# SHI-Labs/Self-Similarity-Grouping

Measured on AMD Instinct MI355X. Metric: images/s embed + s/iter for NxN rerank+DBSCAN, N=16k, 1/2/4/8 GPU, higher is better.
Workload: dtype f32 (embed: split-half operands hi+lo on fp16 MFMA, fp32 accumulate, 6e-8 max error vs the fp32 reference features) / exact int64 via int8 MFMA digits + f64 + f16 (distance, re-rank: half semantics, bit-exact)

## Files before the change

include/ssg_hip.h:

```cpp
#ifndef SSG_HIP_H
#define SSG_HIP_H

#include <stddef.h>
#include <stdint.h>

#ifdef __cplusplus
extern "C" {
#endif

typedef struct ihipStream_t* ssg_stream_t;

#define SSG_OK 0
#define SSG_ERR_INVALID (-1)
#define SSG_ERR_HIP (-2)
#define SSG_ERR_OVERFLOW (-3)
#define SSG_ERR_NAN (-4)

const char* ssg_last_error(void);
int ssg_version(void);
uint16_t ssg_double_to_half_bits(double d);

int ssg_range_stats_f32(const float* a, int rows_a, const float* b, int rows_b, int d, float* out4, ssg_stream_t stream);
int ssg_row_norms_f64(const float* x, int n, int d, int round_to_half, double* norms, ssg_stream_t stream);
int ssg_sqdist_self_f16(const float* x, const double* norms, int N, int d, int row0, int nrows, int memory_save, uint16_t* D, uint32_t* rowmax,
// ... 87 lines not shown
                           const int64_t* seg_off, const int32_t* seg_len, int nseg, const uint64_t* s_cursor, const uint32_t* vmin,
                           uint16_t jp0_half, uint8_t* rowmask, int32_t* cnt, int32_t* edges, uint64_t cap_edges, uint64_t* cursor2,
                           ssg_stream_t stream);
int ssg_concat_segments_u64(const uint64_t* in, int nseg, uint64_t seg_cap, uint64_t seg_stride, const uint64_t* counts, int count_stride,
                            uint64_t* out, uint64_t* total2, ssg_stream_t stream);
size_t ssg_dbscan_cc_workspace_bytes(int N);
int ssg_dbscan_cc(const int32_t* cnt, const int32_t* edges, uint64_t nedges, int N, int min_samples, void* ws, size_t ws_bytes,
                  int64_t* labels, ssg_stream_t stream);
int ssg_dbscan_cc_dev(const int32_t* cnt, const int32_t* edges, const uint64_t* nedges_dev, uint64_t cap_edges, int N, int min_samples,
                      void* ws, size_t ws_bytes, int64_t* labels, ssg_stream_t stream);

int ssg_conv2d_nhwc_f32(const float* in, const float* w, const float* bias, const float* res, float* out, int B, int H, int W, int Cin,
                        int Cout, int KH, int KW, int stride, int pad, int relu, ssg_stream_t stream);
int ssg_conv1x1_dual_nhwc_f32(const float* in, const float* in2, const float* w, const float* bias, float* out, int B, int H, int W, int Cin,
                              int H2, int W2, int Cin2, int stride2, int Cout, int relu, ssg_stream_t stream);
#define SSG_CONV_IN_SPLIT 1
#define SSG_CONV_OUT_SPLIT 2
int ssg_conv2d_nhwc_x(const void* in, const void* w, const float* bias, const void* res, void* out, int B, int H, int W, int Cin,
                      int Cout, int KH, int KW, int stride, int pad, int relu, int flags, float acc_scale, const float* ch_scale,
                      int32_t* overflow, ssg_stream_t stream);
int ssg_conv1x1_dual_nhwc_x(const void* in, const void* in2, const void* w, const float* bias, void* out, int B, int H, int W, int Cin,
                            int H2, int W2, int Cin2, int stride2, int Cout, int relu, int flags, float acc_scale, const float* ch_scale,
                            int32_t* overflow, ssg_stream_t stream);
int ssg_conv_pair_supported(int K1, int C, int N2);
int ssg_conv_pair_nhwc_x(const void* y2, const void* w3, const float* b3, const float* cs3, const void* res, void* out,
                         const void* w1n, const float* b1n, const float* cs1n, void* y1n, int M, int K1, int C, int N2,
                         int32_t* overflow, ssg_stream_t stream);
int ssg_bottleneck_supported(int H, int W, int CIN, int C, int MID);
int ssg_bottleneck_nhwc_x(const void* x, const void* w1, const float* b1, const float* cs1, const void* w2, const float* b2, const float* cs2,
                          const void* w3, const float* b3, const float* cs3, void* out, int B, int H, int W, int C, int MID,
                          int32_t* overflow, ssg_stream_t stream);
int ssg_bottleneck_ds_nhwc_x(const void* x, const void* w1, const float* b1, const float* cs1, const void* w2, const float* b2, const float* cs2,
                             const void* w3cat, const float* b3, const float* cs3, void* out, int B, int H, int W, int CIN, int C, int MID,
                             int32_t* overflow, ssg_stream_t stream);
int ssg_basicblock_supported(int H, int W, int C);
int ssg_basicblock_nhwc_x(const void* x, const void* w1, const float* b1, const float* cs1, const void* w2, const float* b2, const float* cs2,
                          void* out, int B, int H, int W, int C, int32_t* overflow, ssg_stream_t stream);
int ssg_stem_pool_supported(int H, int W);
int ssg_stem_pool_nchw_x(const float* images, int flip, const void* w, const float* bias, const float* ch_scale, void* out, int B, int H, int W,
                         int32_t* overflow, ssg_stream_t stream);
int ssg_nchw_to_nhwc4_h4l4(const float* in, void* out, int B, int H, int W, int flip, ssg_stream_t stream);
int ssg_maxpool3x3s2_h8l8(const void* in, void* out, int B, int H, int W, int C, ssg_stream_t stream);
int ssg_gap_stripes_h8l8(const void* in, float* out, int B, int H, int W, int C, int num_split, ssg_stream_t stream);
int ssg_h8l8_encode(const float* in, void* out, int64_t n, float scale, ssg_stream_t stream);
int ssg_h8l8_decode(const void* in, float* out, int64_t n, float scale, ssg_stream_t stream);
int ssg_pairwise_sqdist_f32(const float* x, const float* y, int m, int n, int d, int self_form, float* ws, float* out, ssg_stream_t stream);
// ... 179 lines not shown
```

self-similarity-grouping_amd/csrc/conv.hip:

```cpp
#include "ssg_common.h"
#include <cstdlib>
#include <type_traits>

namespace ssg {

typedef float v16f __attribute__((ext_vector_type(16)));
typedef unsigned int v4u __attribute__((ext_vector_type(4)));
typedef _Float16 v8h __attribute__((ext_vector_type(8)));

__device__ __forceinline__ unsigned pack_h2(_Float16 a, _Float16 b) {
  return (unsigned)__builtin_bit_cast(unsigned short, a) | ((unsigned)__builtin_bit_cast(unsigned short, b) << 16);
}
__device__ __forceinline__ float unpack_lo(unsigned u) { return (float)__builtin_bit_cast(_Float16, (unsigned short)(u & 0xffffu)); }
__device__ __forceinline__ float unpack_hi(unsigned u) { return (float)__builtin_bit_cast(_Float16, (unsigned short)(u >> 16)); }
__device__ __forceinline__ void split_encode4(const float4 v, uint2& hi, uint2& lo) {
  const _Float16 h0 = (_Float16)v.x, h1 = (_Float16)v.y, h2 = (_Float16)v.z, h3 = (_Float16)v.w;
  hi = make_uint2(pack_h2(h0, h1), pack_h2(h2, h3));
  lo = make_uint2(pack_h2((_Float16)(v.x - (float)h0), (_Float16)(v.y - (float)h1)), pack_h2((_Float16)(v.z - (float)h2), (_Float16)(v.w - (float)h3)));
}
__device__ __forceinline__ bool split_hi_nonfinite(const uint2 hi) {
  const unsigned a = hi.x & 0x7fff7fffu, b = hi.y & 0x7fff7fffu;
  return (a & 0xffffu) >= 0x7c00u || (a >> 16) >= 0x7c00u || (b & 0xffffu) >= 0x7c00u || (b >> 16) >= 0x7c00u;
}
__device__ __forceinline__ float4 split_decode4(const uint2 hi, const uint2 lo) {
  return make_float4(unpack_lo(hi.x) + unpack_lo(lo.x), unpack_hi(hi.x) + unpack_hi(lo.x), unpack_lo(hi.y) + unpack_lo(lo.y), unpack_hi(hi.y) + unpack_hi(lo.y));
}

struct ConvParams {
  const float* in; const float* w; const float* bias; const float* res; float* out;
  int B, H, W, Cin, OH, OW, Cout, KH, KW, stride, pad, relu;
  int M, Kpad;
  int variant;
  unsigned in_bytes;
  const float* in2; int H2, W2, Cin2, stride2, nk1; unsigned in2_bytes;
  const float* rowterm; int epi;
  float* tilemin; int tmin_ld;
  int out_split, res_split; float acc_scale;
  const float* cscale = nullptr;
  int* overflow = nullptr;
  int products = 3;
  unsigned long long* prof = nullptr;
};
#ifdef SSG_DMA_PROF
#define SSG_DMA_STAMP(I_) { if (p.prof && threadIdx.x == 0) p.prof[(size_t)blockIdx.x * 8 + (I_)] = __builtin_readcyclecounter(); }
#else
#define SSG_DMA_STAMP(I_)
#endif

constexpr int CLD32 = 36;

__device__ __forceinline__ int conv_xcd_remap(int b, int nwg) {
  const int nx = 8, q = nwg / nx, r = nwg % nx, x = b % nx, s = b / nx;
  return (x < r ? x * (q + 1) : r * (q + 1) + (x - r) * q) + s;
}

template <int MT, int NT> struct SplitFrags { v8h ah[MT], al[MT], bh[NT], bl[NT]; };

typedef float v4f __attribute__((ext_vector_type(4)));
template <int MT, int NT, int CLD, bool TAP4>
__device__ __forceinline__ void split_load_frags(const float* Arow, const float* Brow, const int kofs, SplitFrags<MT, NT>& f) {
#pragma unroll
  for (int i = 0; i < MT; i++) {
    const float* q = Arow + i * 32 * CLD + kofs;
// ... 406 lines not shown
  const int wm = wave / WCOLS, wn = wave % WCOLS, l32 = lane & 31, h = lane >> 5;

  const int drow = lane >> 2, pc = lane & 3;
  const int lc4 = (pc ^ ((drow >> 2) & 3)) * 4;
  const int nkA = DUAL ? p.nk1 * 2 : 0x7fffffff;
  int ab0, ah0, aw0, ab1 = -1, ah1 = 0, aw1 = 0, abase0 = 0, abase1 = 0;
  unsigned a2b0 = 0x80000000u, a2b1 = 0x80000000u;
#define SSG_ROW(J)                                                                                                   \
  {                                                                                                                  \
    const int m = tm * BM + (wave * ABLK + J) * 16 + drow;                                                            \
    if (m < p.M) {                                                                                                   \
      const int b = m / (p.OH * p.OW), rem = m - b * (p.OH * p.OW);                                                  \
      const int oh = rem / p.OW, ow = rem - oh * p.OW;                                                               \
      ab##J = b; ah##J = oh * p.stride - p.pad; aw##J = ow * p.stride - p.pad;                                       \
      abase##J = (((b * p.H + ah##J) * p.W + aw##J) * p.Cin + lc4) * 4;                                               \
      if (DUAL) a2b##J = (unsigned)((((b * p.H2 + oh * p.stride2) * p.W2 + ow * p.stride2) * p.Cin2 + lc4) * 4);       \
    } else { ab##J = -1; ah##J = 0; aw##J = 0; }                                                                     \
  }
  SSG_ROW(0)
  if (ABLK == 2) SSG_ROW(1)
#undef SSG_ROW
  const __amdgpu_buffer_rsrc_t in_rsrc = __builtin_amdgcn_make_buffer_rsrc(const_cast<float*>(p.in), 0, p.in_bytes, 0x00020000);
  const __amdgpu_buffer_rsrc_t in2_rsrc = __builtin_amdgcn_make_buffer_rsrc(const_cast<float*>(p.in2 ? p.in2 : p.in), 0, p.in2 ? p.in2_bytes : 0u, 0x00020000);
  const __amdgpu_buffer_rsrc_t w_rsrc = __builtin_amdgcn_make_buffer_rsrc(const_cast<float*>(p.w), 0, (unsigned)((int64_t)p.Cout * p.Kpad * 4), 0x00020000);
  const unsigned wo0 = (unsigned)(((tn * BN + wave * (16 * WBLK) + drow) * p.Kpad + lc4) * 4), wo1 = wo0 + (unsigned)(16 * p.Kpad * 4);
  const int nk = p.Kpad / CBK;
  int dn = 0, dr = 0, ds = 0, dch = 0;
#ifndef SSG_DMA_AUX_A
#define SSG_DMA_AUX_A 0
#endif
#ifndef SSG_DMA_AUX_W
#define SSG_DMA_AUX_W 0
#endif
#define SSG_DMA_A(J, ST)                                                                                             \
  {                                                                                                                  \
    if (!DUAL || dn < nkA) {                                                                                          \
      const bool ok = ab##J >= 0 && (unsigned)(ah##J + dr) < (unsigned)p.H && (unsigned)(aw##J + ds) < (unsigned)p.W;  \
      const unsigned aoff = ok ? (unsigned)(abase##J + ddelta_) : 0x80000000u;                                        \
      __builtin_amdgcn_raw_ptr_buffer_load_lds(in_rsrc, SSG_LDSP(ST + (wave * ABLK + J) * 1024), 16, aoff, 0, 0, SSG_DMA_AUX_A);   \
    } else {                                                                                                          \
      const unsigned aoff = a2b##J + (unsigned)((dn - nkA) * CBK * 4);                                                 \
      __builtin_amdgcn_raw_ptr_buffer_load_lds(in2_rsrc, SSG_LDSP(ST + (wave * ABLK + J) * 1024), 16, aoff, 0, 0, SSG_DMA_AUX_A);  \
    }                                                                                                                 \
  }
#define SSG_DMA_NEXT(ST)                                                                                             \
  {                                                                                                                  \
    const int ddelta_ = ((dr * p.W + ds) * p.Cin + dch * 32 + (dn & 1) * 16) * 4;                                     \
    SSG_DMA_A(0, ST) if (ABLK == 2) SSG_DMA_A(1, ST)                                                                  \
    const unsigned kb_ = (unsigned)(dn * CBK * 4);                                                                    \
    __builtin_amdgcn_raw_ptr_buffer_load_lds(w_rsrc, SSG_LDSP(ST + BM * 64 + wave * (1024 * WBLK)), 16, wo0 + kb_, 0, 0, SSG_DMA_AUX_W);   \
    if (WBLK == 2) __builtin_amdgcn_raw_ptr_buffer_load_lds(w_rsrc, SSG_LDSP(ST + BM * 64 + wave * 2048 + 1024), 16, wo1 + kb_, 0, 0, SSG_DMA_AUX_W); \
    {                                         \
      const int adv_ = dn < nk - 1 ? 1 : 0;                                                                          \
      dn += adv_;                                                                                                    \
      ds += adv_ & ~dn & 1;                                                                                          \
      const int w1_ = ds == p.KW ? 1 : 0; ds = w1_ ? 0 : ds; dr += w1_;                                               \
      const int w2_ = dr == p.KH ? 1 : 0; dr = w2_ ? 0 : dr; dch += w2_;                                              \
    }                                                                                                                \
  }

  const int g = (l32 >> 2) & 3;
  const int offh = ((2 * h) ^ g) * 16, offl = ((2 * h + 1) ^ g) * 16;
  const int arow = (wm * WM + l32) * 64, brow = BM * 64 + (wn * WN + l32) * 64;
#define SSG_MMA(ST)                                                                                                  \
  {                                                                                                                  \
    v8h ah_[MT], al_[MT], bh_[NT], bl_[NT];                                                                          \
    _Pragma("unroll") for (int i = 0; i < MT; i++) {                                                                 \
      ah_[i] = *reinterpret_cast<const v8h*>(ST + arow + i * 2048 + offh); al_[i] = *reinterpret_cast<const v8h*>(ST + arow + i * 2048 + offl); } \
    _Pragma("unroll") for (int j = 0; j < NT; j++) {                                                                 \
      bh_[j] = *reinterpret_cast<const v8h*>(ST + brow + j * 2048 + offh); bl_[j] = *reinterpret_cast<const v8h*>(ST + brow + j * 2048 + offl); } \
    if constexpr (!ONEPROD) {                                                                                        \
      _Pragma("unroll") for (int i = 0; i < MT; i++) _Pragma("unroll") for (int j = 0; j < NT; j++)                  \
// ... 310 lines not shown
            const unsigned s0 = odd ? __float_as_uint(r4.x) : __float_as_uint(r4.z), s1 = odd ? __float_as_uint(r4.y) : __float_as_uint(r4.w);
            const unsigned g0 = lane_xor1(s0), g1 = lane_xor1(s1);
            r4 = odd ? split_decode4(make_uint2(g0, g1), make_uint2(__float_as_uint(r4.z), __float_as_uint(r4.w)))
                     : split_decode4(make_uint2(__float_as_uint(r4.x), __float_as_uint(r4.y)), make_uint2(g0, g1));
          }
          v.x += r4.x; v.y += r4.y; v.z += r4.z; v.w += r4.w;
        }
        if (p.relu) { v.x = v.x > 0.f ? v.x : 0.f; v.y = v.y > 0.f ? v.y : 0.f; v.z = v.z > 0.f ? v.z : 0.f; v.w = v.w > 0.f ? v.w : 0.f; }
        if (p.out_split) {
          uint2 hp, lp;
          split_encode4(v, hp, lp);
          if (p.overflow && split_hi_nonfinite(hp)) *p.overflow = 1;
          const uint2 send = odd ? hp : lp;
          const uint2 recv = make_uint2(lane_xor1(send.x), lane_xor1(send.y));
          const uint4 stv = odd ? make_uint4(recv.x, recv.y, lp.x, lp.y) : make_uint4(hp.x, hp.y, recv.x, recv.y);
          if (m < p.M) *reinterpret_cast<uint4*>(outp + (int64_t)m * p.Cout + col) = stv;
        } else if (m < p.M) *reinterpret_cast<float4*>(outp + (int64_t)m * p.Cout + col) = v;
      }
      __builtin_amdgcn_fence(__ATOMIC_ACQ_REL, "wavefront");
    }
  }
}

__global__ void nchw_to_nhwc4_kernel(const float* __restrict__ in, float* __restrict__ out, int B, int H, int W, int flip) {
  const int64_t total = (int64_t)B * H * W;
  for (int64_t x = (int64_t)blockIdx.x * blockDim.x + threadIdx.x; x < total; x += (int64_t)gridDim.x * blockDim.x) {
    const int w = (int)(x % W); const int64_t t = x / W; const int hh = (int)(t % H); const int b = (int)(t / H);
    const int ws = flip ? (W - 1 - w) : w;
    const int64_t plane = (int64_t)H * W, base = (int64_t)b * 3 * plane + (int64_t)hh * W + ws;
    reinterpret_cast<float4*>(out)[x] = make_float4(in[base], in[base + plane], in[base + 2 * plane], 0.f);
  }
}

__global__ void nchw_to_nhwc4_h4l4_kernel(const float* __restrict__ in, float* __restrict__ out, int B, int H, int W, int flip) {
  const int64_t total = (int64_t)B * H * W;
  for (int64_t x = (int64_t)blockIdx.x * blockDim.x + threadIdx.x; x < total; x += (int64_t)gridDim.x * blockDim.x) {
    const int w = (int)(x % W); const int64_t t = x / W; const int hh = (int)(t % H); const int b = (int)(t / H);
    const int ws = flip ? (W - 1 - w) : w;
    const int64_t plane = (int64_t)H * W, base = (int64_t)b * 3 * plane + (int64_t)hh * W + ws;
    uint2 hi, lo;
    split_encode4(make_float4(in[base], in[base + plane], in[base + 2 * plane], 0.f), hi, lo);
    reinterpret_cast<uint4*>(out)[x] = make_uint4(hi.x, hi.y, lo.x, lo.y);
  }
}

__global__ void maxpool3x3s2_kernel(const float* __restrict__ in, float* __restrict__ out, int B, int H, int W, int C, int OH, int OW) {
// ... 183 lines not shown
      if (tall_wm == 128) hipLaunchKernelGGL((conv_dma_kernel<256, false, 256, false, 4, 128, false>), dim3(tiles_tall), dim3(512), 0, stream, p);
      else if (tall_wm == 129) hipLaunchKernelGGL((conv_dma_kernel<256, false, 256, false, 4, 128, true>), dim3(tiles_tall), dim3(512), 0, stream, p);
      else if (tall_ns == 4) hipLaunchKernelGGL((conv_dma_kernel<256, false, 256, false, 4>), dim3(tiles_tall), dim3(1024), 0, stream, p);
      else hipLaunchKernelGGL((conv_dma_kernel<256, false, 256, false>), dim3(tiles_tall), dim3(1024), 0, stream, p);
      return ssg_check_hip(hipGetLastError(), "conv_dma_kernel<256x256>");
    }
    const int tiles = ((p.M + 127) / 128) * (p.Cout / 256);
    if (p.products == 1) hipLaunchKernelGGL((conv_dma_kernel<256, true>), dim3(tiles), dim3(512), 0, stream, p);
    else if (p.in2) hipLaunchKernelGGL((conv_dma_kernel<256, false, 128, true>), dim3(tiles), dim3(512), 0, stream, p);
    else hipLaunchKernelGGL(conv_dma_kernel<256>, dim3(tiles), dim3(512), 0, stream, p);
    return ssg_check_hip(hipGetLastError(), "conv_dma_kernel");
  }
  return launch_conv_bk<128, 256, 64, 64, false, 32, true>(p, stream);
}

static bool conv_prefers_bn64(const ConvParams& p, bool split) {
  static int maxtiles = -1;
  if (maxtiles < 0) { const char* e = getenv("SSG_SPLIT_BN64_MAXTILES"); maxtiles = e ? atoi(e) : 300; }
  if (!split) return false;
  const int tiles = ((p.M + 127) / 128) * (p.Cout / 128);
  return tiles < maxtiles;
}

extern "C" int ssg_conv2d_nhwc_x(const void* in, const void* w, const float* bias, const void* res, void* out, int B, int H, int W,
                                 int Cin, int Cout, int KH, int KW, int stride, int pad, int relu, int flags, float acc_scale, const float* ch_scale,
                                 int32_t* overflow, hipStream_t stream) {
  ConvParams p;
  p.cscale = ch_scale; p.overflow = overflow;
  p.in = (const float*)in; p.w = (const float*)w; p.bias = bias; p.res = (const float*)res; p.out = (float*)out;
  p.B = B; p.H = H; p.W = W; p.Cin = Cin; p.Cout = Cout; p.KH = KH; p.KW = KW; p.stride = stride; p.pad = pad; p.relu = relu;
  p.OH = (H + 2 * pad - KH) / stride + 1; p.OW = (W + 2 * pad - KW) / stride + 1;
  const int64_t M = (int64_t)B * p.OH * p.OW;
  const bool split = (flags & 1) != 0;
  if (B <= 0 || M <= 0 || M > 0x7fffffff || (Cout % 64) || !((Cin % 32) == 0 || Cin == 4) || stride < 1) {
    ssg_set_error("ssg_conv2d_nhwc: unsupported shape B=%d H=%d W=%d Cin=%d Cout=%d k=%dx%d s=%d p=%d flags=%d", B, H, W, Cin, Cout, KH, KW, stride, pad, flags);
    return SSG_ERR_INVALID;
  }
  p.M = (int)M;
  const int64_t in_bytes = (int64_t)B * H * W * Cin * 4;
  if (in_bytes > 0x7fffffffLL) { ssg_set_error("ssg_conv2d_nhwc: input tensor of %lld bytes exceeds the 2 GiB buffer-resource range of this kernel; use a smaller batch", (long long)in_bytes); return SSG_ERR_INVALID; }
  p.in_bytes = (unsigned)in_bytes;
  p.in2 = nullptr; p.H2 = p.W2 = p.Cin2 = 0; p.stride2 = 1; p.in2_bytes = 0; p.rowterm = nullptr; p.epi = 0; p.tilemin = nullptr; p.tmin_ld = 0;
  p.out_split = (flags & 2) ? 1 : 0; p.res_split = p.out_split; p.acc_scale = acc_scale;
  static int variant = -1;
  if (variant < 0) { const char* e = getenv("SSG_CONV_VARIANT"); variant = e ? atoi(e) : 0; }
  p.variant = variant;
  const bool cin4 = (Cin == 4);
  p.Kpad = cin4 ? 32 * ((KH * KW + 7) / 8) : KH * KW * Cin;
  p.nk1 = p.Kpad / 16;
  if (cin4) return (Cout % 128 == 0) ? launch_conv<128, 128, 64, 64, true>(p, stream, split) : launch_conv<128, 64, 64, 32, true>(p, stream, split);
  if (conv_prefers_wide(p, split)) return launch_conv_wide(p, stream);
  return (Cout % 128 == 0 && !conv_prefers_bn64(p, split)) ? launch_conv<128, 128, 64, 64, false>(p, stream, split) : launch_conv<128, 64, 64, 32, false>(p, stream, split);
}

extern "C" int ssg_conv2d_nhwc_f32(const float* in, const float* w, const float* bias, const float* res, float* out, int B, int H, int W,
                                   int Cin, int Cout, int KH, int KW, int stride, int pad, int relu, hipStream_t stream) {
  return ssg_conv2d_nhwc_x(in, w, bias, res, out, B, H, W, Cin, Cout, KH, KW, stride, pad, relu, 0, 1.f, nullptr, nullptr, stream);
}

extern "C" int ssg_conv1x1_dual_nhwc_x(const void* in, const void* in2, const void* w, const float* bias, void* out, int B, int H, int W,
                                       int Cin, int H2, int W2, int Cin2, int stride2, int Cout, int relu, int flags, float acc_scale, const float* ch_scale,
                                       int32_t* overflow, hipStream_t stream) {
  ConvParams p;
  p.cscale = ch_scale; p.overflow = overflow;
  p.in = (const float*)in; p.w = (const float*)w; p.bias = bias; p.res = nullptr; p.out = (float*)out;
  p.B = B; p.H = H; p.W = W; p.Cin = Cin; p.Cout = Cout; p.KH = 1; p.KW = 1; p.stride = 1; p.pad = 0; p.relu = relu;
  p.OH = H; p.OW = W;
  const int64_t M = (int64_t)B * H * W;
  const int64_t in_bytes = M * Cin * 4, in2_bytes = (int64_t)B * H2 * W2 * Cin2 * 4;
  if (B <= 0 || M > 0x7fffffff || (Cout % 64) || (Cin % 32) || (Cin2 % 32) || stride2 < 1 || (H - 1) * stride2 >= H2 || (W - 1) * stride2 >= W2 ||
      in_bytes > 0x7fffffffLL || in2_bytes > 0x7fffffffLL) {
    ssg_set_error("ssg_conv1x1_dual_nhwc: unsupported shape B=%d H=%d W=%d Cin=%d H2=%d W2=%d Cin2=%d s2=%d Cout=%d", B, H, W, Cin, H2, W2, Cin2, stride2, Cout);
    return SSG_ERR_INVALID;
  }
  p.M = (int)M; p.in_bytes = (unsigned)in_bytes;
  p.in2 = (const float*)in2; p.H2 = H2; p.W2 = W2; p.Cin2 = Cin2; p.stride2 = stride2; p.in2_bytes = (unsigned)in2_bytes;
  p.Kpad = Cin + Cin2; p.nk1 = Cin / 32; p.variant = 0; p.rowterm = nullptr; p.epi = 0; p.tilemin = nullptr; p.tmin_ld = 0;
  p.out_split = (flags & 2) ? 1 : 0; p.res_split = p.out_split; p.acc_scale = acc_scale;
  const bool split = (flags & 1) != 0;
  if (conv_prefers_wide(p, split)) return launch_conv_wide(p, stream);
  return (Cout % 128 == 0 && !conv_prefers_bn64(p, split)) ? launch_conv<128, 128, 64, 64, false>(p, stream, split) : launch_conv<128, 64, 64, 32, false>(p, stream, split);
}

extern "C" int ssg_conv1x1_dual_nhwc_f32(const float* in, const float* in2, const float* w, const float* bias, float* out, int B, int H, int W,
                                         int Cin, int H2, int W2, int Cin2, int stride2, int Cout, int relu, hipStream_t stream) {
  return ssg_conv1x1_dual_nhwc_x(in, in2, w, bias, out, B, H, W, Cin, H2, W2, Cin2, stride2, Cout, relu, 0, 1.f, nullptr, nullptr, stream);
}

namespace ssg {
__global__ __launch_bounds__(256) void row_sqnorm_kernel(const float* __restrict__ x, int rows, int d, float scale, float* __restrict__ out) {
  const int row = (int)((blockIdx.x * blockDim.x + threadIdx.x) >> 6);
  if (row >= rows) return;
  const int lane = lane_id();
  float s = 0.f;
  const float* xr = x + (int64_t)row * d;
  for (int c0 = lane; c0 < d; c0 += 512) {
    float v[8];
#pragma unroll
    for (int u = 0; u < 8; u++) v[u] = xr[min(c0 + 64 * u, d - 1)];
#pragma unroll
    for (int u = 0; u < 8; u++) if (c0 + 64 * u < d) s += v[u] * v[u];
  }
  for (int sh = 1; sh < 64; sh <<= 1) s += __shfl_xor(s, sh, 64);
  if (lane == 0) out[row] = s * scale;
// ... 98 lines not shown
```

self-similarity-grouping_amd/resnet.py:

```python
from collections import OrderedDict

import math
import os

import torch

from . import _lib
from ._lib import check, ptr, stream

_LAYERS = {18: (2, 2, 2, 2), 34: (3, 4, 6, 3), 50: (3, 4, 6, 3), 101: (3, 4, 23, 3), 152: (3, 8, 36, 3)}
_BASIC = (18, 34)
_BN_EPS = 1e-5
_DEC_CLUSTERS, _DEC_DIM, _DEC_KEY = 32, 2048, "assignment.cluster_centers"
_FUSED_BASICBLOCK_DEFAULT = "1"


def _expansion(depth):
    return 1 if depth in _BASIC else 4


def _arch(depth):
    blocks = []
    inplanes = 64
    exp = _expansion(depth)
# ... 35 lines not shown
            conv(p + ".conv2", pl, pl, 3); bn(p + ".bn2", pl)
            if blk["down"]:
                conv(p + ".downsample.0", pl, ip, 1); bn(p + ".downsample.1", pl)
            continue
        conv(p + ".conv1", pl, ip, 1); bn(p + ".bn1", pl)
        conv(p + ".conv2", pl, pl, 3); bn(p + ".bn2", pl)
        conv(p + ".conv3", pl * 4, pl, 1); bn(p + ".bn3", pl * 4)
        if blk["down"]:
            conv(p + ".downsample.0", pl * 4, ip, 1); bn(p + ".downsample.1", pl * 4)
    sd["base.fc.weight"] = torch.randn(1000, width, generator=g) * 0.01
    sd["base.fc.bias"] = torch.zeros(1000)
    if num_features > 0:
        sd["feat.weight"] = torch.randn(num_features, width, generator=g) * 0.001
        sd["feat_bn.weight"] = torch.ones(num_features); sd["feat_bn.bias"] = torch.zeros(num_features)
        sd["feat_bn.running_mean"] = torch.zeros(num_features); sd["feat_bn.running_var"] = torch.ones(num_features)
        sd["feat_bn.num_batches_tracked"] = torch.zeros((), dtype=torch.long)
    if cluster:
        bound = math.sqrt(6.0 / (_DEC_CLUSTERS + _DEC_DIM))
        sd[_DEC_KEY] = (torch.rand(_DEC_CLUSTERS, _DEC_DIM, generator=g) * 2.0 - 1.0) * bound
    return sd


class _FoldedConv:
    __slots__ = ("w", "bias", "cin", "cout", "k", "stride", "pad", "split", "acc_scale", "cscale")


_IN_SPLIT, _OUT_SPLIT = 1, 2


def _h8l8(v):
    rows, K = v.shape
    hi = v.half()
    lo = (v - hi.float()).half()
    g = torch.stack([hi.view(rows, K // 8, 8), lo.view(rows, K // 8, 8)], dim=2)
    return g.reshape(rows, 2 * K).contiguous().view(torch.float32)


def _h4l4(v):
    rows, K = v.shape
    hi = v.half()
    lo = (v - hi.float()).half()
    g = torch.stack([hi.view(rows, K // 4, 4), lo.view(rows, K // 4, 4)], dim=2)
    return g.reshape(rows, 2 * K).contiguous().view(torch.float32)


def _weight_scale(w):
    mx = float(w.abs().max())
    return 256.0 if mx == 0 else float(min(256.0, 2.0 ** math.floor(math.log2(16384.0 / mx))))


# ... 15 lines not shown
    mean, var = sd[bn_name + ".running_mean"].double(), sd[bn_name + ".running_var"].double()
    scale = gamma / torch.sqrt(var + _BN_EPS)
    w = w * scale.view(-1, 1, 1, 1)
    bias = beta - mean * scale
    cout, cin, k, _ = w.shape
    w = w.permute(0, 2, 3, 1).contiguous()
    if cin == 3:
        w = torch.nn.functional.pad(w, (0, 1))
        cin = 4
        kpad = 32 * ((k * k + 7) // 8)
        w = torch.nn.functional.pad(w.reshape(cout, k * k * 4), (0, kpad - k * k * 4))
    else:
        w = pack_weight_khwc(w)
    f = _FoldedConv()
    w = w.float().contiguous()
    f.split, f.acc_scale, f.cscale = bool(split), 1.0, None
    if split:
        sc = _row_scales(w)
        w = w * sc.view(-1, 1)
        w = _h4l4(w) if cin == 4 else _h8l8(w)
        f.cscale = (1.0 / sc).contiguous().to(device)
    f.w = w.to(device); f.bias = bias.float().contiguous().to(device)
    f.cin, f.cout, f.k, f.stride, f.pad = cin, cout, k, stride, pad
    return f


def _fold_mode():
    return os.environ.get("SSG_DEVICE_FOLD", "")


def _bn_keys(conv_name, bn_name):
    return (conv_name + ".weight", bn_name + ".weight", bn_name + ".bias", bn_name + ".running_mean", bn_name + ".running_var")


def _use_device_fold(sd, keys):
    mode = _fold_mode()
    return mode == "1" or (mode != "0" and any(sd[k].device.type != "cpu" for k in keys))


def _fold_device(sources, stride, pad, device, split=False):
    L = _lib.lib()
    srcs = [[t.detach().to(device, torch.float32) for t in s] for s in sources]
    w = srcs[0][0]
    cout, cin, k, kw = w.shape
    f = _FoldedConv()
    f.split, f.acc_scale, f.cscale = bool(split), 1.0, None
    kp = 32 * ((k * kw + 7) // 8) if cin == 3 else sum(s[0].shape[1] * s[0].shape[2] * s[0].shape[3] for s in srcs)
    f.w = torch.empty((cout, kp), dtype=torch.float32, device=device)
    f.bias = torch.empty(cout, dtype=torch.float32, device=device)
    if split:
        f.cscale = torch.empty(cout, dtype=torch.float32, device=device)
    if len(srcs) == 1:
        g, b, m, v = srcs[0][1:]
        st = w.stride()
        check(L.ssg_fold_conv_bn_f32(ptr(w), st[0], st[1], st[2], st[3], cout, cin, k, kw, ptr(g), ptr(b), ptr(m), ptr(v), _BN_EPS, 1 if split else 0,
                                     ptr(f.w), ptr(f.bias), ptr(f.cscale), stream()), "ssg_fold_conv_bn_f32")
    else:
        args = []
        for wt, g, b, m, v in srcs:
            st = wt.stride()
            args += [ptr(wt), st[0], st[1], st[2], st[3], wt.shape[1], wt.shape[2], wt.shape[3], ptr(g), ptr(b), ptr(m), ptr(v)]
        check(L.ssg_fold_conv_bn_dual_f32(*args, _BN_EPS, cout, 1 if split else 0, ptr(f.w), ptr(f.bias), ptr(f.cscale), stream()),
              "ssg_fold_conv_bn_dual_f32")
    last = srcs[-1][0]
    f.cin, f.cout, f.k, f.stride, f.pad = (4 if cin == 3 else last.shape[1]), cout, last.shape[2], stride, pad
    return f


class ResNet:

    def __init__(self, depth=50, checkpoint=None, pretrained=True, num_features=2048, dropout=0.1, num_classes=0, num_split=1,
                 mode='Dissimilarity', cluster=False, seed=1, precision=None):
        if depth not in _LAYERS:
            raise KeyError("Unsupported depth:", depth)
        if num_classes > 0:
            raise NotImplementedError("num_classes > 0 (dropout + classifier head, resnet.py:118-120) is a training-only path; "
                                      "the grouping path uses num_classes=0 (selftraining.py:121-123)")
        if num_features > 0 and num_features % 64:
            raise ValueError("num_features must be a multiple of 64")
        self.depth, self.num_features, self.dropout, self.num_classes = depth, num_features, dropout, num_classes
        self.out_planes = 512 * _expansion(depth)
        self.num_split, self.cluster, self.pretrained, self.training = num_split, cluster, pretrained, False
        self.precision = precision or os.environ.get("SSG_EMBED_PRECISION", "split")
        if self.precision not in ("split", "f32"):
            raise ValueError("precision must be 'split' or 'f32'")
        self.device = torch.device("cpu")
        self._sd = synthetic_state_dict(seed, depth, num_features, cluster=bool(cluster))
        self._folded = None
        self._twin = None
        self.flip_streams = True
        self._weights = "synthetic"
        if checkpoint:
            self.load_state_dict(torch.load(checkpoint, map_location="cpu"), strict=False)
        elif pretrained:
            import warnings
            warnings.warn("ssg_amd ResNet(pretrained=True): no ImageNet weights are available offline; the backbone holds seeded "
                          "synthetic weights until load_state_dict()/checkpoint= supplies real ones", stacklevel=2)

    def state_dict(self):
        return OrderedDict((k, v.clone() if v.device.type == "cpu" else v.cpu()) for k, v in self._sd.items())

    def load_state_dict(self, state_dict, strict=True):
        state_dict, missing, unexpected = self._match_keys(state_dict, strict)
        for k, v in state_dict.items():
            if k in self._sd:
                if tuple(v.shape) != tuple(self._sd[k].shape):
                    raise RuntimeError("size mismatch for %s: %r vs %r" % (k, tuple(v.shape), tuple(self._sd[k].shape)))
                self._sd[k] = v.detach().to("cpu").clone()
        self._invalidate()
        self._report_missing("load_state_dict", missing)
        return missing, unexpected

# ... 68 lines not shown
    def _host_sd(self, keys):
        return {k: self._sd[k].cpu() for k in keys}

    def _fold_one(self, conv_name, bn_name, stride, pad, split=False):
        keys = _bn_keys(conv_name, bn_name)
        if _use_device_fold(self._sd, keys):
            return _fold_device([[self._sd[k] for k in keys]], stride, pad, self.device, split=split)
        return _fold(self._host_sd(keys), conv_name, bn_name, stride, pad, self.device, split=split)

    def _fold_dual(self, p, stride, sp):
        dev = self.device
        k3, kd = _bn_keys(p + ".conv3", p + ".bn3"), _bn_keys(p + ".downsample.0", p + ".downsample.1")
        if _use_device_fold(self._sd, k3 + kd):
            c3 = _fold_device([[self._sd[k] for k in k3]], 1, 0, dev)
            ds = _fold_device([[self._sd[k] for k in k3], [self._sd[k] for k in kd]], stride, 0, dev, split=sp)
            return c3, ds
        sd = self._host_sd(k3 + kd)
        c3 = _fold(sd, p + ".conv3", p + ".bn3", 1, 0, dev)
        ds = _fold(sd, p + ".downsample.0", p + ".downsample.1", stride, 0, dev)
        wcat = torch.cat([c3.w, ds.w], dim=1)
        if sp:
            sc = _row_scales(wcat.cpu())
            ds.w = _h8l8((wcat.cpu() * sc.view(-1, 1))).to(dev); ds.acc_scale = 1.0; ds.cscale = (1.0 / sc).contiguous().to(dev); ds.split = True
        else:
            ds.w = wcat.contiguous()
        ds.bias = (c3.bias + ds.bias).contiguous()
        return c3, ds

    def _prepare(self):
        if self._folded is not None:
            return self._folded
        if self.device.type != "cuda":
            raise _lib.SSGError("the embedder runs on the GPU only: call model.cuda() first (no CPU fallback)")
        sp = self.precision == "split"
        fold = self._fold_one
        net = dict(stem=fold("base.conv1", "base.bn1", 2, 3, sp), blocks=[], split=sp)
        for blk in _arch(self.depth):
            p = blk["prefix"]
            if blk["kind"] == "basic":
                net["blocks"].append(dict(
                    kind="basic",
                    c1=fold(p + ".conv1", p + ".bn1", blk["stride"], 1, sp),
                    c2=fold(p + ".conv2", p + ".bn2", 1, 1, sp),
                    ds=fold(p + ".downsample.0", p + ".downsample.1", blk["stride"], 0, sp) if blk["down"] else None))
                continue
            if blk["down"]:
                c3, ds = self._fold_dual(p, blk["stride"], sp)
            else:
                c3, ds = fold(p + ".conv3", p + ".bn3", 1, 0, sp), None
            net["blocks"].append(dict(
                c1=fold(p + ".conv1", p + ".bn1", 1, 0, sp),
                c2=fold(p + ".conv2", p + ".bn2", blk["stride"], 1, sp),
                c3=c3, ds=ds))
        self._folded = net
        return net

    @staticmethod
    def _conv(L, x, f, res=None, relu=True, out_split=False, ovf=None):
        B, H, W, _ = x.shape
        OH = (H + 2 * f.pad - f.k) // f.stride + 1; OW = (W + 2 * f.pad - f.k) // f.stride + 1
        out = torch.empty((B, OH, OW, f.cout), dtype=torch.float32, device=x.device)
        flags = (_IN_SPLIT if f.split else 0) | (_OUT_SPLIT if out_split else 0)
        check(L.ssg_conv2d_nhwc_x(ptr(x), ptr(f.w), ptr(f.bias), ptr(res), ptr(out), B, H, W, f.cin, f.cout, f.k, f.k, f.stride, f.pad,
                                  1 if relu else 0, flags, f.acc_scale, ptr(getattr(f, "cscale", None)), ptr(ovf), stream()), "ssg_conv2d_nhwc_x")
        return out

    @staticmethod
    def _conv_dual(L, o, x, c3, ds, out_split=False, ovf=None):
        B, H, W, _ = o.shape
        _, H2, W2, _ = x.shape
        out = torch.empty((B, H, W, c3.cout), dtype=torch.float32, device=o.device)
        flags = (_IN_SPLIT if ds.split else 0) | (_OUT_SPLIT if out_split else 0)
        check(L.ssg_conv1x1_dual_nhwc_x(ptr(o), ptr(x), ptr(ds.w), ptr(ds.bias), ptr(out), B, H, W, c3.cin, H2, W2, ds.cin, ds.stride, c3.cout, 1,
                                        flags, ds.acc_scale, ptr(getattr(ds, "cscale", None)), ptr(ovf), stream()), "ssg_conv1x1_dual_nhwc_x")
        return out

    @staticmethod
    def _bottleneck(L, y, blk, ovf=None):
        B, H, W, CIN = y.shape
        c1, c2, c3, ds = blk["c1"], blk["c2"], blk["c3"], blk["ds"]
        if os.environ.get("SSG_FUSED_BOTTLENECK", "1") == "0" or c2.stride != 1 or (ds is not None and ds.stride != 1):
            return None
        if not L.ssg_bottleneck_supported(H, W, CIN, c3.cout, c1.cout):
            return None
        out = torch.empty((B, H, W, c3.cout), dtype=torch.float32, device=y.device)
        if ds is None:
            check(L.ssg_bottleneck_nhwc_x(ptr(y), ptr(c1.w), ptr(c1.bias), ptr(c1.cscale), ptr(c2.w), ptr(c2.bias), ptr(c2.cscale),
                                          ptr(c3.w), ptr(c3.bias), ptr(c3.cscale), ptr(out), B, H, W, CIN, c1.cout, ptr(ovf), stream()),
                  "ssg_bottleneck_nhwc_x")
        else:
            check(L.ssg_bottleneck_ds_nhwc_x(ptr(y), ptr(c1.w), ptr(c1.bias), ptr(c1.cscale), ptr(c2.w), ptr(c2.bias), ptr(c2.cscale),
                                             ptr(ds.w), ptr(ds.bias), ptr(ds.cscale), ptr(out), B, H, W, CIN, c3.cout, c1.cout, ptr(ovf), stream()),
                  "ssg_bottleneck_ds_nhwc_x")
        return out

    @staticmethod
    def _basicblock(L, y, blk, ovf=None):
        B, H, W, C = y.shape
        c1, c2 = blk["c1"], blk["c2"]
        if os.environ.get("SSG_FUSED_BASICBLOCK", _FUSED_BASICBLOCK_DEFAULT) == "0" or c1.stride != 1 or blk["ds"] is not None or c1.cout != C:
            return None
        if not L.ssg_basicblock_supported(H, W, C):
            return None
        out = torch.empty((B, H, W, C), dtype=torch.float32, device=y.device)
        check(L.ssg_basicblock_nhwc_x(ptr(y), ptr(c1.w), ptr(c1.bias), ptr(c1.cscale), ptr(c2.w), ptr(c2.bias), ptr(c2.cscale), ptr(out),
                                      B, H, W, C, ptr(ovf), stream()), "ssg_basicblock_nhwc_x")
        return out

    def _fmap(self, x, flip=False, hooks=None):
        L = _lib.lib()
        net = self._prepare()
        sp = net["split"]
        x = x.to(self.device, torch.float32).contiguous()
        B, C, H, W = x.shape
        if C != 3:
            raise ValueError("expected RGB images [B,3,H,W]")
        ovf = self._overflow_flag() if sp else None
        if sp and os.environ.get("SSG_FUSED_STEM", "1") != "0" and L.ssg_stem_pool_supported(H, W):
            st = net["stem"]
            y = torch.empty((B, H // 4, W // 4, 64), dtype=torch.float32, device=self.device)
            check(L.ssg_stem_pool_nchw_x(ptr(x), 1 if flip else 0, ptr(st.w), ptr(st.bias), ptr(st.cscale), ptr(y), B, H, W, ptr(ovf), stream()),
                  "ssg_stem_pool_nchw_x")
        else:
            x4 = torch.empty((B, H, W, 4), dtype=torch.float32, device=self.device)
            if sp:
                check(L.ssg_nchw_to_nhwc4_h4l4(ptr(x), ptr(x4), B, H, W, 1 if flip else 0, stream()), "ssg_nchw_to_nhwc4_h4l4")
            else:
                check(L.ssg_nchw_to_nhwc4(ptr(x), ptr(x4), B, H, W, 1 if flip else 0, stream()), "ssg_nchw_to_nhwc4")
            y = self._conv(L, x4, net["stem"], out_split=sp, ovf=ovf)
            _, H2, W2, _ = y.shape
            p = torch.empty((B, (H2 + 1) // 2, (W2 + 1) // 2, 64), dtype=torch.float32, device=self.device)
            if sp:
                check(L.ssg_maxpool3x3s2_h8l8(ptr(y), ptr(p), B, H2, W2, 64, stream()), "ssg_maxpool3x3s2_h8l8")
            else:
                check(L.ssg_maxpool3x3s2_nhwc(ptr(y), ptr(p), B, H2, W2, 64, stream()), "ssg_maxpool3x3s2_nhwc")
            y = p
        pair = sp and os.environ.get("SSG_CONV_PAIR", "0") == "1"
        blocks, o1_next = net["blocks"], None
        for bi, blk in enumerate(blocks):
            if hooks and bi in hooks:
                hooks[bi]()
            if blk.get("kind") == "basic":
                fused = self._basicblock(L, y, blk, ovf) if sp else None
                if fused is not None:
                    y = fused
                    continue
                o = self._conv(L, y, blk["c1"], out_split=sp, ovf=ovf)
                r = y if blk["ds"] is None else self._conv(L, y, blk["ds"], relu=False, out_split=sp, ovf=ovf)
                y = self._conv(L, o, blk["c2"], res=r, relu=True, out_split=sp, ovf=ovf)
                continue
            if sp:
                fused = self._bottleneck(L, y, blk, ovf)
                if fused is not None:
                    y = fused
                    continue
            o = o1_next if o1_next is not None else self._conv(L, y, blk["c1"], out_split=sp, ovf=ovf)
            o1_next = None
            o = self._conv(L, o, blk["c2"], out_split=sp, ovf=ovf)
            if blk["ds"] is not None:
                y = self._conv_dual(L, o, y, blk["c3"], blk["ds"], out_split=sp, ovf=ovf)
                continue
            nxt = blocks[bi + 1]["c1"] if bi + 1 < len(blocks) else None
            Bo, Ho, Wo, _ = o.shape
            if (pair and nxt is not None and nxt.k == 1 and nxt.stride == 1 and nxt.cin == blk["c3"].cout and Bo * Ho * Wo >= 128 * 256
                    and L.ssg_conv_pair_supported(blk["c3"].cin, blk["c3"].cout, nxt.cout)):
                y, o1_next = self._conv_pair(L, o, blk["c3"], y, nxt, ovf)
            else:
                y = self._conv(L, o, blk["c3"], res=y, relu=True, out_split=sp, ovf=ovf)
        return y, sp

    @staticmethod
    def _conv_pair(L, o, c3, res, c1n, ovf=None):
        B, H, W, _ = o.shape
        out = torch.empty((B, H, W, c3.cout), dtype=torch.float32, device=o.device)
        y1n = torch.empty((B, H, W, c1n.cout), dtype=torch.float32, device=o.device)
        check(L.ssg_conv_pair_nhwc_x(ptr(o), ptr(c3.w), ptr(c3.bias), ptr(c3.cscale), ptr(res), ptr(out), ptr(c1n.w), ptr(c1n.bias), ptr(c1n.cscale),
                                     ptr(y1n), B * H * W, c3.cin, c3.cout, c1n.cout, ptr(ovf), stream()), "ssg_conv_pair_nhwc_x")
        return out, y1n

    def _side_streams(self):
        st = getattr(self, "_streams", None)
        if st is None or st[0].device != self.device:
            prio = -1 if os.environ.get("SSG_FLIP_PRIO", "0") == "1" else 0
            st = self._streams = (torch.cuda.Stream(self.device, priority=prio), torch.cuda.Stream(self.device))
        return st

    def _overflow_flag(self):
        if getattr(self, "_ovf", None) is None or self._ovf.device != self.device:
            self._ovf = torch.zeros(1, dtype=torch.int32, device=self.device)
        return self._ovf

# ... 157 lines not shown
```

Before: 27860.

## Pre-tile conv weights into swizzled 128-row K-tile blocks for contiguous DMA loads

Adds a one-time kernel that rearranges split-half conv weights into 128-output-channel by K-tile blocks, with an XOR swizzle on the 16-byte columns. The conv kernel reads this copy through the buffer-to-LDS loads, so each wave fetches one contiguous 1 KiB chunk per K step instead of strided rows. The tiled copy sits right after the original weights in one allocation, and the python path sets a flag so the kernel finds it at w + Cout*Kpad. This costs double the weight memory and a tiling pass at fold time, and only applies to split-half weights with Cout divisible by 128.

```diff
diff --git a/include/ssg_hip.h b/include/ssg_hip.h
--- a/include/ssg_hip.h
+++ b/include/ssg_hip.h
@@ -133,6 +133,15 @@
 int ssg_conv1x1_dual_nhwc_x(const void* in, const void* in2, const void* w, const float* bias, void* out, int B, int H, int W, int Cin,
                             int H2, int W2, int Cin2, int stride2, int Cout, int relu, int flags, float acc_scale, const float* ch_scale,
                             int32_t* overflow, ssg_stream_t stream);
+#define SSG_CONV_W_TILED 4
+int ssg_conv_weights_tile_supported(int Cout, int Kpad);
+int ssg_conv_weights_tile(const void* w, int Cout, int Kpad, void* wt, ssg_stream_t stream);
+int ssg_conv2d_nhwc_xt(const void* in, const void* w, const void* wt, const float* bias, const void* res, void* out, int B, int H, int W, int Cin,
+                       int Cout, int KH, int KW, int stride, int pad, int relu, int flags, float acc_scale, const float* ch_scale,
+                       int32_t* overflow, ssg_stream_t stream);
+int ssg_conv1x1_dual_nhwc_xt(const void* in, const void* in2, const void* w, const void* wt, const float* bias, void* out, int B, int H, int W, int Cin,
+                             int H2, int W2, int Cin2, int stride2, int Cout, int relu, int flags, float acc_scale, const float* ch_scale,
+                             int32_t* overflow, ssg_stream_t stream);
 int ssg_conv_pair_supported(int K1, int C, int N2);
 int ssg_conv_pair_nhwc_x(const void* y2, const void* w3, const float* b3, const float* cs3, const void* res, void* out,
                          const void* w1n, const float* b1n, const float* cs1n, void* y1n, int M, int K1, int C, int N2,
diff --git a/self-similarity-grouping_amd/csrc/conv.hip b/self-similarity-grouping_amd/csrc/conv.hip
--- a/self-similarity-grouping_amd/csrc/conv.hip
+++ b/self-similarity-grouping_amd/csrc/conv.hip
@@ -39,6 +39,7 @@
   const float* cscale = nullptr;
   int* overflow = nullptr;
   int products = 3;
+  const float* wt = nullptr;
   unsigned long long* prof = nullptr;
 };
 #ifdef SSG_DMA_PROF
@@ -491,9 +492,16 @@
 #undef SSG_ROW
   const __amdgpu_buffer_rsrc_t in_rsrc = __builtin_amdgcn_make_buffer_rsrc(const_cast<float*>(p.in), 0, p.in_bytes, 0x00020000);
   const __amdgpu_buffer_rsrc_t in2_rsrc = __builtin_amdgcn_make_buffer_rsrc(const_cast<float*>(p.in2 ? p.in2 : p.in), 0, p.in2 ? p.in2_bytes : 0u, 0x00020000);
-  const __amdgpu_buffer_rsrc_t w_rsrc = __builtin_amdgcn_make_buffer_rsrc(const_cast<float*>(p.w), 0, (unsigned)((int64_t)p.Cout * p.Kpad * 4), 0x00020000);
-  const unsigned wo0 = (unsigned)(((tn * BN + wave * (16 * WBLK) + drow) * p.Kpad + lc4) * 4), wo1 = wo0 + (unsigned)(16 * p.Kpad * 4);
+#ifndef SSG_CONV_WT
+#define SSG_CONV_WT 1
+#endif
   const int nk = p.Kpad / CBK;
+  const bool tiled = SSG_CONV_WT && !ONEPROD && p.wt != nullptr;
+  const __amdgpu_buffer_rsrc_t w_rsrc = __builtin_amdgcn_make_buffer_rsrc(const_cast<float*>(tiled ? p.wt : p.w), 0, (unsigned)((int64_t)p.Cout * p.Kpad * 4), 0x00020000);
+  const int wrow0 = tn * BN + wave * (16 * WBLK);
+  const unsigned wo0 = tiled ? (unsigned)((((wrow0 >> 7) * nk) * 128 + (wrow0 & 127)) * 64 + lane * 16) : (unsigned)(((wrow0 + drow) * p.Kpad + lc4) * 4);
+  const unsigned wo1 = wo0 + (tiled ? 1024u : (unsigned)(16 * p.Kpad * 4));
+  const int wkshift = tiled ? 13 : 6;
   int dn = 0, dr = 0, ds = 0, dch = 0;
 #ifndef SSG_DMA_AUX_A
 #define SSG_DMA_AUX_A 0
@@ -516,7 +524,7 @@
   {                                                                                                                  \
     const int ddelta_ = ((dr * p.W + ds) * p.Cin + dch * 32 + (dn & 1) * 16) * 4;                                     \
     SSG_DMA_A(0, ST) if (ABLK == 2) SSG_DMA_A(1, ST)                                                                  \
-    const unsigned kb_ = (unsigned)(dn * CBK * 4);                                                                    \
+    const unsigned kb_ = (unsigned)dn << wkshift;                                                                     \
     __builtin_amdgcn_raw_ptr_buffer_load_lds(w_rsrc, SSG_LDSP(ST + BM * 64 + wave * (1024 * WBLK)), 16, wo0 + kb_, 0, 0, SSG_DMA_AUX_W);   \
     if (WBLK == 2) __builtin_amdgcn_raw_ptr_buffer_load_lds(w_rsrc, SSG_LDSP(ST + BM * 64 + wave * 2048 + 1024), 16, wo1 + kb_, 0, 0, SSG_DMA_AUX_W); \
     {                                         \
@@ -873,6 +881,16 @@
   }
 }
 
+__global__ __launch_bounds__(256) void conv_weights_tile_kernel(const uint4* __restrict__ w, uint4* __restrict__ wt, int nk, int64_t nslots) {
+  const int64_t s = (int64_t)blockIdx.x * 256 + threadIdx.x;
+  if (s >= nslots) return;
+  const int64_t gran = s >> 9;
+  const int row = (int)(s >> 2) & 127, pc = (int)s & 3;
+  const int64_t gc = gran / nk; const int kt = (int)(gran - gc * nk);
+  const int lc = pc ^ ((row >> 2) & 3);
+  wt[s] = w[((gc * 128 + row) * nk + kt) * 4 + lc];
+}
+
 __global__ void nchw_to_nhwc4_kernel(const float* __restrict__ in, float* __restrict__ out, int B, int H, int W, int flip) {
   const int64_t total = (int64_t)B * H * W;
   for (int64_t x = (int64_t)blockIdx.x * blockDim.x + threadIdx.x; x < total; x += (int64_t)gridDim.x * blockDim.x) {
@@ -1102,9 +1120,30 @@
   return tiles < maxtiles;
 }
 
-extern "C" int ssg_conv2d_nhwc_x(const void* in, const void* w, const float* bias, const void* res, void* out, int B, int H, int W,
-                                 int Cin, int Cout, int KH, int KW, int stride, int pad, int relu, int flags, float acc_scale, const float* ch_scale,
-                                 int32_t* overflow, hipStream_t stream) {
+extern "C" int ssg_conv_weights_tile_supported(int Cout, int Kpad) { return Cout > 0 && Kpad > 0 && Cout % 128 == 0 && Kpad % 16 == 0; }
+
+extern "C" int ssg_conv_weights_tile(const void* w, int Cout, int Kpad, void* wt, hipStream_t stream) {
+  if (!ssg_conv_weights_tile_supported(Cout, Kpad)) return 0;
+  if (!w || !wt || (((uintptr_t)w | (uintptr_t)wt) & 15)) { ssg_set_error("ssg_conv_weights_tile: w and wt must be given and 16-byte aligned"); return SSG_ERR_INVALID; }
+  const int64_t nslots = (int64_t)Cout * Kpad / 4;
+  hipLaunchKernelGGL(conv_weights_tile_kernel, dim3((unsigned)((nslots + 255) / 256)), dim3(256), 0, stream, (const uint4*)w, (uint4*)wt, Kpad / 16, nslots);
+  SSG_LAUNCH_CHECK("conv_weights_tile_kernel");
+  return 1;
+}
+
+static const void* conv_tiled_weights(const char* fn, const void* w, const void* wt, int flags, int Cout, int64_t Kpad, int* rc) {
+  *rc = SSG_OK;
+  if (!wt && (flags & 4)) wt = (const float*)w + (int64_t)Cout * Kpad;
+  if (wt && (!(flags & 1) || !ssg_conv_weights_tile_supported(Cout, (int)Kpad))) {
+    ssg_set_error("%s: tiled weights need split-half operands, Cout %% 128 == 0 and Kpad %% 16 == 0 (Cout=%d Kpad=%lld flags=%d)", fn, Cout, (long long)Kpad, flags);
+    *rc = SSG_ERR_INVALID;
+  }
+  return wt;
+}
+
+extern "C" int ssg_conv2d_nhwc_xt(const void* in, const void* w, const void* wt, const float* bias, const void* res, void* out, int B, int H, int W,
+                                  int Cin, int Cout, int KH, int KW, int stride, int pad, int relu, int flags, float acc_scale, const float* ch_scale,
+                                  int32_t* overflow, hipStream_t stream) {
   ConvParams p;
   p.cscale = ch_scale; p.overflow = overflow;
   p.in = (const float*)in; p.w = (const float*)w; p.bias = bias; p.res = (const float*)res; p.out = (float*)out;
@@ -1128,19 +1167,26 @@
   const bool cin4 = (Cin == 4);
   p.Kpad = cin4 ? 32 * ((KH * KW + 7) / 8) : KH * KW * Cin;
   p.nk1 = p.Kpad / 16;
+  { int rc; p.wt = (const float*)conv_tiled_weights("ssg_conv2d_nhwc_xt", w, wt, flags, Cout, p.Kpad, &rc); if (rc) return rc; }
   if (cin4) return (Cout % 128 == 0) ? launch_conv<128, 128, 64, 64, true>(p, stream, split) : launch_conv<128, 64, 64, 32, true>(p, stream, split);
   if (conv_prefers_wide(p, split)) return launch_conv_wide(p, stream);
   return (Cout % 128 == 0 && !conv_prefers_bn64(p, split)) ? launch_conv<128, 128, 64, 64, false>(p, stream, split) : launch_conv<128, 64, 64, 32, false>(p, stream, split);
 }
 
+extern "C" int ssg_conv2d_nhwc_x(const void* in, const void* w, const float* bias, const void* res, void* out, int B, int H, int W,
+                                 int Cin, int Cout, int KH, int KW, int stride, int pad, int relu, int flags, float acc_scale, const float* ch_scale,
+                                 int32_t* overflow, hipStream_t stream) {
+  return ssg_conv2d_nhwc_xt(in, w, nullptr, bias, res, out, B, H, W, Cin, Cout, KH, KW, stride, pad, relu, flags, acc_scale, ch_scale, overflow, stream);
+}
+
 extern "C" int ssg_conv2d_nhwc_f32(const float* in, const float* w, const float* bias, const float* res, float* out, int B, int H, int W,
                                    int Cin, int Cout, int KH, int KW, int stride, int pad, int relu, hipStream_t stream) {
   return ssg_conv2d_nhwc_x(in, w, bias, res, out, B, H, W, Cin, Cout, KH, KW, stride, pad, relu, 0, 1.f, nullptr, nullptr, stream);
 }
 
-extern "C" int ssg_conv1x1_dual_nhwc_x(const void* in, const void* in2, const void* w, const float* bias, void* out, int B, int H, int W,
-                                       int Cin, int H2, int W2, int Cin2, int stride2, int Cout, int relu, int flags, float acc_scale, const float* ch_scale,
-                                       int32_t* overflow, hipStream_t stream) {
+extern "C" int ssg_conv1x1_dual_nhwc_xt(const void* in, const void* in2, const void* w, const void* wt, const float* bias, void* out, int B, int H, int W,
+                                        int Cin, int H2, int W2, int Cin2, int stride2, int Cout, int relu, int flags, float acc_scale, const float* ch_scale,
+                                        int32_t* overflow, hipStream_t stream) {
   ConvParams p;
   p.cscale = ch_scale; p.overflow = overflow;
   p.in = (const float*)in; p.w = (const float*)w; p.bias = bias; p.res = nullptr; p.out = (float*)out;
@@ -1158,8 +1204,15 @@
   p.Kpad = Cin + Cin2; p.nk1 = Cin / 32; p.variant = 0; p.rowterm = nullptr; p.epi = 0; p.tilemin = nullptr; p.tmin_ld = 0;
   p.out_split = (flags & 2) ? 1 : 0; p.res_split = p.out_split; p.acc_scale = acc_scale;
   const bool split = (flags & 1) != 0;
+  { int rc; p.wt = (const float*)conv_tiled_weights("ssg_conv1x1_dual_nhwc_xt", w, wt, flags, Cout, p.Kpad, &rc); if (rc) return rc; }
   if (conv_prefers_wide(p, split)) return launch_conv_wide(p, stream);
   return (Cout % 128 == 0 && !conv_prefers_bn64(p, split)) ? launch_conv<128, 128, 64, 64, false>(p, stream, split) : launch_conv<128, 64, 64, 32, false>(p, stream, split);
+}
+
+extern "C" int ssg_conv1x1_dual_nhwc_x(const void* in, const void* in2, const void* w, const float* bias, void* out, int B, int H, int W,
+                                       int Cin, int H2, int W2, int Cin2, int stride2, int Cout, int relu, int flags, float acc_scale, const float* ch_scale,
+                                       int32_t* overflow, hipStream_t stream) {
+  return ssg_conv1x1_dual_nhwc_xt(in, in2, w, nullptr, bias, out, B, H, W, Cin, H2, W2, Cin2, stride2, Cout, relu, flags, acc_scale, ch_scale, overflow, stream);
 }
 
 extern "C" int ssg_conv1x1_dual_nhwc_f32(const float* in, const float* in2, const float* w, const float* bias, float* out, int B, int H, int W,
diff --git a/self-similarity-grouping_amd/resnet.py b/self-similarity-grouping_amd/resnet.py
--- a/self-similarity-grouping_amd/resnet.py
+++ b/self-similarity-grouping_amd/resnet.py
@@ -81,10 +81,27 @@
 
 
 class _FoldedConv:
-    __slots__ = ("w", "bias", "cin", "cout", "k", "stride", "pad", "split", "acc_scale", "cscale")
-
-
-_IN_SPLIT, _OUT_SPLIT = 1, 2
+    __slots__ = ("w", "bias", "cin", "cout", "k", "stride", "pad", "split", "acc_scale", "cscale", "wt")
+
+
+_IN_SPLIT, _OUT_SPLIT, _W_TILED = 1, 2, 4
+
+
+def _attach_tiled(f):
+    f.wt = None
+    cout, kp = f.w.shape
+    if not f.split or f.cin == 4 or f.w.device.type != "cuda":
+        return f
+    L = _lib.lib()
+    if not L.ssg_conv_weights_tile_supported(cout, kp):
+        return f
+    both = torch.empty((2, cout, kp), dtype=torch.float32, device=f.w.device)
+    both[0].copy_(f.w)
+    rc = L.ssg_conv_weights_tile(ptr(both[0]), cout, kp, ptr(both[1]), stream())
+    if rc != 1:
+        check(rc if rc < 0 else -2, "ssg_conv_weights_tile")
+    f.w, f.wt = both[0], both[1]
+    return f
 
 
 def _h8l8(v):
@@ -146,7 +163,7 @@
         f.cscale = (1.0 / sc).contiguous().to(device)
     f.w = w.to(device); f.bias = bias.float().contiguous().to(device)
     f.cin, f.cout, f.k, f.stride, f.pad = cin, cout, k, stride, pad
-    return f
+    return _attach_tiled(f)
 
 
 def _fold_mode():
@@ -188,7 +205,7 @@
               "ssg_fold_conv_bn_dual_f32")
     last = srcs[-1][0]
     f.cin, f.cout, f.k, f.stride, f.pad = (4 if cin == 3 else last.shape[1]), cout, last.shape[2], stride, pad
-    return f
+    return _attach_tiled(f)
 
 
 class ResNet:
@@ -212,6 +229,7 @@
         self._sd = synthetic_state_dict(seed, depth, num_features, cluster=bool(cluster))
         self._folded = None
         self._twin = None
+        self.tiled_weights = os.environ.get("SSG_CONV_WT", "1") != "0"
         self.flip_streams = True
         self._weights = "synthetic"
         if checkpoint:
@@ -326,6 +344,7 @@
         if sp:
             sc = _row_scales(wcat.cpu())
             ds.w = _h8l8((wcat.cpu() * sc.view(-1, 1))).to(dev); ds.acc_scale = 1.0; ds.cscale = (1.0 / sc).contiguous().to(dev); ds.split = True
+            _attach_tiled(ds)
         else:
             ds.w = wcat.contiguous()
         ds.bias = (c3.bias + ds.bias).contiguous()
@@ -360,21 +379,21 @@
         return net
 
     @staticmethod
-    def _conv(L, x, f, res=None, relu=True, out_split=False, ovf=None):
+    def _conv(L, x, f, res=None, relu=True, out_split=False, ovf=None, tiled=False):
         B, H, W, _ = x.shape
         OH = (H + 2 * f.pad - f.k) // f.stride + 1; OW = (W + 2 * f.pad - f.k) // f.stride + 1
         out = torch.empty((B, OH, OW, f.cout), dtype=torch.float32, device=x.device)
-        flags = (_IN_SPLIT if f.split else 0) | (_OUT_SPLIT if out_split else 0)
+        flags = (_IN_SPLIT if f.split else 0) | (_OUT_SPLIT if out_split else 0) | (_W_TILED if tiled and f.wt is not None else 0)
         check(L.ssg_conv2d_nhwc_x(ptr(x), ptr(f.w), ptr(f.bias), ptr(res), ptr(out), B, H, W, f.cin, f.cout, f.k, f.k, f.stride, f.pad,
                                   1 if relu else 0, flags, f.acc_scale, ptr(getattr(f, "cscale", None)), ptr(ovf), stream()), "ssg_conv2d_nhwc_x")
         return out
 
     @staticmethod
-    def _conv_dual(L, o, x, c3, ds, out_split=False, ovf=None):
+    def _conv_dual(L, o, x, c3, ds, out_split=False, ovf=None, tiled=False):
         B, H, W, _ = o.shape
         _, H2, W2, _ = x.shape
         out = torch.empty((B, H, W, c3.cout), dtype=torch.float32, device=o.device)
-        flags = (_IN_SPLIT if ds.split else 0) | (_OUT_SPLIT if out_split else 0)
+        flags = (_IN_SPLIT if ds.split else 0) | (_OUT_SPLIT if out_split else 0) | (_W_TILED if tiled and ds.wt is not None else 0)
         check(L.ssg_conv1x1_dual_nhwc_x(ptr(o), ptr(x), ptr(ds.w), ptr(ds.bias), ptr(out), B, H, W, c3.cin, H2, W2, ds.cin, ds.stride, c3.cout, 1,
                                         flags, ds.acc_scale, ptr(getattr(ds, "cscale", None)), ptr(ovf), stream()), "ssg_conv1x1_dual_nhwc_x")
         return out
@@ -415,6 +434,7 @@
         L = _lib.lib()
         net = self._prepare()
         sp = net["split"]
+        tw = bool(getattr(self, "tiled_weights", True))
         x = x.to(self.device, torch.float32).contiguous()
         B, C, H, W = x.shape
         if C != 3:
@@ -449,20 +469,20 @@
                 if fused is not None:
                     y = fused
                     continue
-                o = self._conv(L, y, blk["c1"], out_split=sp, ovf=ovf)
-                r = y if blk["ds"] is None else self._conv(L, y, blk["ds"], relu=False, out_split=sp, ovf=ovf)
-                y = self._conv(L, o, blk["c2"], res=r, relu=True, out_split=sp, ovf=ovf)
+                o = self._conv(L, y, blk["c1"], out_split=sp, ovf=ovf, tiled=tw)
+                r = y if blk["ds"] is None else self._conv(L, y, blk["ds"], relu=False, out_split=sp, ovf=ovf, tiled=tw)
+                y = self._conv(L, o, blk["c2"], res=r, relu=True, out_split=sp, ovf=ovf, tiled=tw)
                 continue
             if sp:
                 fused = self._bottleneck(L, y, blk, ovf)
                 if fused is not None:
                     y = fused
                     continue
-            o = o1_next if o1_next is not None else self._conv(L, y, blk["c1"], out_split=sp, ovf=ovf)
+            o = o1_next if o1_next is not None else self._conv(L, y, blk["c1"], out_split=sp, ovf=ovf, tiled=tw)
             o1_next = None
-            o = self._conv(L, o, blk["c2"], out_split=sp, ovf=ovf)
+            o = self._conv(L, o, blk["c2"], out_split=sp, ovf=ovf, tiled=tw)
             if blk["ds"] is not None:
-                y = self._conv_dual(L, o, y, blk["c3"], blk["ds"], out_split=sp, ovf=ovf)
+                y = self._conv_dual(L, o, y, blk["c3"], blk["ds"], out_split=sp, ovf=ovf, tiled=tw)
                 continue
             nxt = blocks[bi + 1]["c1"] if bi + 1 < len(blocks) else None
             Bo, Ho, Wo, _ = o.shape
@@ -470,7 +490,7 @@
                     and L.ssg_conv_pair_supported(blk["c3"].cin, blk["c3"].cout, nxt.cout)):
                 y, o1_next = self._conv_pair(L, o, blk["c3"], y, nxt, ovf)
             else:
-                y = self._conv(L, o, blk["c3"], res=y, relu=True, out_split=sp, ovf=ovf)
+                y = self._conv(L, o, blk["c3"], res=y, relu=True, out_split=sp, ovf=ovf, tiled=tw)
         return y, sp
 
     @staticmethod
```

Result: faster. 28520, median of 6 (+2.4%).
